# mcahny/vps

Measured on NVIDIA H100. Metric: FuseTrack frame pairs/s on synthetic 1024x2048 pairs, higher is better.
Workload: dtype f32 (wgmma: 3 split-f16 products per MAC, fp32 accumulate promoted to RN register sums)

## Files before the change

### vps_b200/csrc/conv_tc32.cu

```cuda
#include "conv_tc_common.cuh"

namespace {

constexpr int T32_CONV_WARPS = 3;
constexpr int T32_KC = 32;
constexpr int T32_MAX_N = 128;
constexpr int T32_WIDE_MAX_N = 64;
constexpr int t32_threads(int nwg) { return 128 * (nwg + 1); }
constexpr int T32_STAGE_SLOTS = 2;
constexpr int T32_PLANES = 2;

__device__ unsigned int g_tc32_overflow = 0;

struct Tc32Extra {
  int rows;
  int plane_bytes;
  int stage_bytes;
  int b_plane_bytes;
  int dcn;
  int dcn_split_n;
};

struct Dcn32Params {
  const float* x;
// ... 11 lines not shown
              "setmaxnreg counts are multiples of 8 in [24, 256]");

struct Ring32 {
  uint32_t s_base, s_bytes;
  uint32_t a_base, a_bytes;
  uint32_t b_base, b_bytes;
  uint32_t e_base, bias_base;
  uint32_t bar_base;
  __device__ __forceinline__ uint32_t sfull(int s) const { return bar_base + 8u * s; }
  __device__ __forceinline__ uint32_t sempty(int s) const { return bar_base + 8u * (MAX_STAGES + s); }
  __device__ __forceinline__ uint32_t pfull(int s) const { return bar_base + 8u * (2 * MAX_STAGES + s); }
  __device__ __forceinline__ uint32_t pempty(int s) const { return bar_base + 8u * (3 * MAX_STAGES + s); }
  __device__ __forceinline__ uint32_t bfull(int s) const { return bar_base + 8u * (4 * MAX_STAGES + s); }
  __device__ __forceinline__ uint32_t bempty(int s) const { return bar_base + 8u * (5 * MAX_STAGES + s); }
  __device__ __forceinline__ uint32_t unit_ctr() const { return bar_base + 8u * (6 * MAX_STAGES); }
  __device__ __forceinline__ uint32_t rfull(int wg) const { return bar_base + 8u * (6 * MAX_STAGES + 1 + wg); }
};
constexpr int T32_NBAR = 6 * MAX_STAGES;
constexpr int T32_BAR_BYTES = 8 * (T32_NBAR + 2 + 4);
constexpr int t32_box_c(int n) { return n >= 32 ? 32 : 16; }
constexpr int T32_EPI_MAX_N = 64;
constexpr int t32_epi_bytes(int nwg, int bn) { return 64 * nwg * bn * 4 + nwg * bn * 4; }

__device__ __forceinline__ void producer32(const ConvTcParams& p, const Tc32Extra& e, const Ring32& rg, const CUtensorMap* tmA,
                                           const CUtensorMap* tmB) {
  const int ntaps = p.kh * p.kw, kw = p.kw;
  const bool halo = p.halo != 0;
  const uint32_t a_box_bytes = (uint32_t)p.a_box_bytes, b_bytes = (uint32_t)T32_PLANES * (uint32_t)e.b_plane_bytes;
  const int bn = p.block_n;
  int ss = 0, bs = 0;
  uint32_t sphase = 0, bphase = 0;
  for (int tile = blockIdx.x; tile < p.total_tiles; tile += gridDim.x) {
    const TileCoord t = tile_coord(p, tile);
    const int x_base = t.tx * p.tw * p.sw - p.pw_[t.prob];
    const int y_base = t.ty * p.th * p.sh - p.ph_[t.prob];
    const int n0 = t.n_idx * bn;
    for (int cc = 0; cc < p.cin_chunks; ++cc) {
      int r = 0, s = 0;
      for (int tap = 0; tap < ntaps; ++tap) {
        if (!e.dcn && (!halo || tap == 0)) {
          mbar_wait(rg.sempty(ss), sphase ^ 1);
          if (elect_one()) {
            mbar_expect_tx(rg.sfull(ss), a_box_bytes);
            tma_load_4d(rg.s_base + ss * rg.s_bytes, tmA, rg.sfull(ss), cc * T32_KC, halo ? x_base : x_base + s,
                        halo ? y_base : y_base + r, t.img);
          }
          if (++ss == T32_STAGE_SLOTS) { ss = 0; sphase ^= 1; }
        }
        mbar_wait(rg.bempty(bs), bphase ^ 1);
        if (elect_one()) {
          mbar_expect_tx(rg.bfull(bs), b_bytes);
          tma_load_5d(rg.b_base + bs * rg.b_bytes, tmB, rg.bfull(bs), cc * T32_KC, n0, tap, t.prob, 0);
        }
        if (++bs == p.b_stages) { bs = 0; bphase ^= 1; }
        if (++s == kw) { s = 0; ++r; }
      }
    }
  }
}

__device__ __forceinline__ void converter32(const ConvTcParams& p, const Tc32Extra& e, const Ring32& rg, int ctid, int nthreads) {
  const int ntaps = p.kh * p.kw;
  const int items_per_tile = p.cin_chunks * (p.halo ? 1 : ntaps);
  const int tasks = e.rows * 4;
  int ss = 0, as = 0;
  uint32_t sphase = 0, aphase = 0;
  bool over = false;
  for (int tile = blockIdx.x; tile < p.total_tiles; tile += gridDim.x) {
    for (int it = 0; it < items_per_tile; ++it) {
      mbar_wait(rg.sfull(ss), sphase);
      mbar_wait(rg.pempty(as), aphase ^ 1);
      const uint32_t src = rg.s_base + ss * rg.s_bytes;
      const uint32_t dst = rg.a_base + as * rg.a_bytes;
      for (int task = ctid; task < tasks; task += nthreads) {
        const int r = task >> 2, j = task & 3;
        const uint32_t row_s = src + (uint32_t)r * 128u;
        const uint32_t sw = (uint32_t)(r & 7);
        float v[8];
        asm volatile("ld.shared.v4.f32 {%0, %1, %2, %3}, [%4];" : "=f"(v[0]), "=f"(v[1]), "=f"(v[2]), "=f"(v[3])
                     : "r"(row_s + (((uint32_t)(2 * j) ^ sw) << 4)));
        asm volatile("ld.shared.v4.f32 {%0, %1, %2, %3}, [%4];" : "=f"(v[4]), "=f"(v[5]), "=f"(v[6]), "=f"(v[7])
                     : "r"(row_s + (((uint32_t)(2 * j + 1) ^ sw) << 4)));
        uint32_t hp[4], lp[4];
#pragma unroll
        for (int q = 0; q < 4; ++q) split_pair_f16(v[2 * q], v[2 * q + 1], hp[q], lp[q], over);
        const uint32_t off = (uint32_t)r * 64u + ((((uint32_t)j) ^ ((uint32_t)(r >> 1) & 3u)) << 4);
        const uint32_t pm = dst + off, pl = pm + (uint32_t)e.plane_bytes;
        asm volatile("st.shared.v4.b32 [%0], {%1, %2, %3, %4};" ::"r"(pm), "r"(hp[0]), "r"(hp[1]), "r"(hp[2]), "r"(hp[3]) : "memory");
        asm volatile("st.shared.v4.b32 [%0], {%1, %2, %3, %4};" ::"r"(pl), "r"(lp[0]), "r"(lp[1]), "r"(lp[2]), "r"(lp[3]) : "memory");
      }
      mbar_arrive(rg.sempty(ss));
      asm volatile("fence.proxy.async.shared::cta;" ::: "memory");
      mbar_arrive(rg.pfull(as));
      if (++ss == T32_STAGE_SLOTS) { ss = 0; sphase ^= 1; }
      if (++as == p.a_stages) { as = 0; aphase ^= 1; }
    }
  }
  if (over) atomicAdd(&g_tc32_overflow, 1u);
}


__device__ __forceinline__ void dcn_gather32(const ConvTcParams& p, const Tc32Extra& e, const Dcn32Params& d, const Ring32& rg,
                                             uint32_t setup_base, uint32_t ctr_addr, int gtid) {
  constexpr int NT = 32 * DCN32_GATHER_WARPS;
  const int lane = gtid & 31;
  const int j = lane & 3;
  const int rlog = e.rows == 128 ? 7 : 6, ulog = rlog - 3;
  const int steps_per_tile = p.cin_chunks * 9;
  const uint32_t units_per_tile = (uint32_t)steps_per_tile << ulog;
  const uint32_t a_stages = (uint32_t)p.a_stages;
  uint32_t step_base = 0;
  for (int tile = blockIdx.x; tile < p.total_tiles; tile += gridDim.x) {
    const TileCoord t = tile_coord(p, tile);
    if (gtid == 0) asm volatile("st.volatile.shared.u32 [%0], %1;" ::"r"(ctr_addr), "r"(0u) : "memory");
    for (int item = gtid; item < 9 << rlog; item += NT) {
      const int k = item >> rlog, r = item & ((1 << rlog) - 1);
      const int ty_in = r / p.tw, tx_in = r - ty_in * p.tw;
      dcn_setup_entry(d, setup_base + (uint32_t)item * 32u, t.img, t.ty * p.th + ty_in, t.tx * p.tw + tx_in, k);
// ... 85 lines not shown
  for (int h = 0; h < 2; ++h) {
    const int q = 16 * w + (lane >> 2) + 8 * h;
#pragma unroll
    for (int j = 0; j < N / 8; ++j) {
      const int c = 8 * j + 2 * (lane & 3);
      const uint32_t a = epi_box_addr<N>(box, q, c);
      float b0, b1, r0 = 0.f, r1 = 0.f;
      asm volatile("ld.shared.v2.f32 {%0, %1}, [%2];" : "=f"(b0), "=f"(b1) : "r"(bias_s + 4u * c));
      if (p.res) asm volatile("ld.shared.v2.f32 {%0, %1}, [%2];" : "=f"(r0), "=f"(r1) : "r"(a));
      const float2 v = epi_math(p, d[4 * j + 2 * h], d[4 * j + 2 * h + 1], b0, b1, r0, r1);
      asm volatile("st.shared.v2.f32 [%0], {%1, %2};" ::"r"(a), "f"(v.x), "f"(v.y) : "memory");
    }
  }
  asm volatile("fence.proxy.async.shared::cta;" ::: "memory");
  asm volatile("bar.sync %0, 128;" ::"r"(1 + wg) : "memory");
  const EpiBox eb = epi_box(p, tile, wg);
  if (i == 0 && eb.live) {
#pragma unroll
    for (int b = 0; b < N / BC; ++b) tma_store_4d(tmY, box + (uint32_t)b * (64u * BC * 4u), eb.n0 + b * BC, eb.x0, eb.y0, eb.img);
    asm volatile("cp.async.bulk.commit_group;" ::: "memory");
  }
}

template <int N, bool TMA_EPI>
__device__ __forceinline__ void consumer32(const ConvTcParams& p, const Tc32Extra& e, const Ring32& rg, int wg, int row0,
                                           uint32_t b_off, int c_off, const CUtensorMap* tmY, const CUtensorMap* tmR) {
  constexpr int BC = t32_box_c(N);
  const bool leader = (threadIdx.x & 127) == 0;
  constexpr bool epi_tma = TMA_EPI;
  const uint32_t box = rg.e_base + (uint32_t)wg * (64u * N * 4u), bias_s = rg.bias_base + (uint32_t)wg * (N * 4u);
  const uint32_t rbar = rg.rfull(wg);
  uint32_t rphase = 0;
  const bool halo = p.halo != 0;
  const int ntaps = p.kh * p.kw, kw = p.kw, last_cc = p.cin_chunks - 1;
  const uint32_t a_pitch = halo ? (uint32_t)p.halo_w * 64u : 512u;
  const uint64_t a_hi = desc_hi(64u, a_pitch), b_hi = desc_hi(64u, 512u);
  const uint32_t a_wg = halo ? (uint32_t)(row0 >> 3) * a_pitch : (uint32_t)row0 * 64u;
  const uint32_t plane = (uint32_t)e.plane_bytes, b_plane = (uint32_t)e.b_plane_bytes;
  float acc[N / 2], sum[N / 2];
  int as = 0, bs = 0;
  uint32_t aphase = 0, bphase = 0;
  for (int tile = blockIdx.x; tile < p.total_tiles; tile += gridDim.x) {
    float bias_v = 0.f;
    if (epi_tma) {
      const int c = tile_coord(p, tile).n_idx * N + (threadIdx.x & 127);
      if (p.bias && (threadIdx.x & 127) < N && c < p.cout) bias_v = __ldg(p.bias + c);
    }
#pragma unroll
    for (int i = 0; i < N / 2; ++i) sum[i] = 0.f;
    for (int cc = 0; cc <= last_cc; ++cc) {
      const bool two = cc != last_cc || p.nk_last > 1;
      uint32_t a_item = 0;
      int r = 0, s = 0;
      for (int tap = 0; tap < ntaps; ++tap) {
        if (!halo || tap == 0) {
          mbar_wait(rg.pfull(as), aphase);
          a_item = rg.a_base + as * rg.a_bytes + a_wg;
        }
        mbar_wait(rg.bfull(bs), bphase);
        const uint32_t a_addr = halo ? a_item + (uint32_t)r * a_pitch + (uint32_t)s * 64u : a_item;
        const uint32_t b_addr = rg.b_base + bs * rg.b_bytes + b_off;
        const uint64_t A = desc_at(a_hi, a_addr), A2 = desc_at(a_hi, a_addr + plane);
        const uint64_t B = desc_at(b_hi, b_addr), B2 = desc_at(b_hi, b_addr + b_plane);
        wg::fence();
        wg::Mma<N, true>::run(acc, A2, B, 0u);
        if (two) wg::Mma<N, true>::run(acc, A2 + 2, B + 2, 1u);
        wg::Mma<N, true>::run(acc, A, B2, 1u);
        if (two) wg::Mma<N, true>::run(acc, A + 2, B2 + 2, 1u);
        wg::commit();
        wg::wait<0>();
        wg::fence_regs(acc);
#pragma unroll
        for (int i = 0; i < N / 2; ++i) acc[i] *= T32_LO_INV;
        wg::fence();
        wg::Mma<N, true>::run(acc, A, B, 1u);
        if (two) wg::Mma<N, true>::run(acc, A + 2, B + 2, 1u);
        wg::commit();
        wg::wait<0>();
        wg::fence_regs(acc);
#pragma unroll
        for (int i = 0; i < N / 2; ++i) sum[i] += acc[i];
        const bool item_done = !halo || tap == ntaps - 1;
        if (leader) {
          mbar_arrive(rg.bempty(bs));
          if (item_done) mbar_arrive(rg.pempty(as));
          if (epi_tma && p.res && cc == 0 && tap == 0) {
            asm volatile("cp.async.bulk.wait_group.read 0;" ::: "memory");
            const EpiBox eb = epi_box(p, tile, wg);
            if (eb.live) {
              mbar_expect_tx(rbar, 64u * N * 4u);
#pragma unroll
              for (int b = 0; b < N / BC; ++b)
                tma_load_4d(box + (uint32_t)b * (64u * BC * 4u), tmR, rbar, eb.n0 + b * BC, eb.x0, eb.y0, eb.img);
            } else {
              mbar_arrive(rbar);
            }
          }
        }
        if (item_done && ++as == p.a_stages) { as = 0; aphase ^= 1; }
        if (++bs == p.b_stages) { bs = 0; bphase ^= 1; }
        if (++s == kw) { s = 0; ++r; }
      }
    }
    if (epi_tma) {
      epi_tma32<N>(p, tmY, sum, box, bias_s, bias_v, rbar, rphase, wg, tile);
      if (p.res) rphase ^= 1u;
    } else {
      epi_frag<N, 4>(p, sum, tile, row0, c_off);
    }
  }
  if (epi_tma && leader) asm volatile("cp.async.bulk.wait_group 0;" ::: "memory");
}

template <int NWG, bool TMA_EPI>
__device__ __forceinline__ void consumer32_n(const ConvTcParams& p, const Tc32Extra& e, const Ring32& rg, int wg,
                                             const CUtensorMap* tmY, const CUtensorMap* tmR) {
  switch (p.block_n) {
    case 16: consumer32<16, TMA_EPI>(p, e, rg, wg, 64 * wg, 0u, 0, tmY, tmR); break;
    case 32: consumer32<32, TMA_EPI>(p, e, rg, wg, 64 * wg, 0u, 0, tmY, tmR); break;
    case 64: consumer32<64, TMA_EPI>(p, e, rg, wg, 64 * wg, 0u, 0, tmY, tmR); break;
    default:
      if constexpr (NWG == 2 && !TMA_EPI) consumer32<T32_MAX_N, false>(p, e, rg, wg, 64 * wg, 0u, 0, tmY, tmR);
      else __trap();
      break;
  }
}

__device__ __forceinline__ void init_bars32(const Ring32& rg, uint32_t pfull_count, uint32_t sempty_count, uint32_t consumers) {
  for (int i = threadIdx.x & 31; i < T32_NBAR; i += 32) {
    const int kind = i / MAX_STAGES;
    const uint32_t count = kind == 1 ? sempty_count : (kind == 2 ? pfull_count : ((kind == 3 || kind == 5) ? consumers : 1u));
    mbar_init(rg.bar_base + 8u * i, count);
  }
  if ((threadIdx.x & 31) < 4) mbar_init(rg.rfull(threadIdx.x & 31), 1u);
  asm volatile("fence.mbarrier_init.release.cluster;" ::: "memory");
}

template <int NWG, bool TMA_EPI>
__global__ void __launch_bounds__(t32_threads(NWG), 1)
conv_igemm_tc32_kernel(const __grid_constant__ CUtensorMap tmA, const __grid_constant__ CUtensorMap tmB,
                       const __grid_constant__ CUtensorMap tmY, const __grid_constant__ CUtensorMap tmR, const ConvTcParams p,
                       const Tc32Extra e) {
  extern __shared__ __align__(1024) uint8_t smem_raw[];
  const uint32_t smem_base = (smem_u32(smem_raw) + 1023u) & ~1023u;
  Ring32 rg;
  rg.s_base = smem_base; rg.s_bytes = (uint32_t)e.stage_bytes;
  rg.a_base = rg.s_base + T32_STAGE_SLOTS * rg.s_bytes; rg.a_bytes = (uint32_t)T32_PLANES * (uint32_t)e.plane_bytes;
  rg.b_base = rg.a_base + (uint32_t)p.a_stages * rg.a_bytes; rg.b_bytes = (uint32_t)T32_PLANES * (uint32_t)e.b_plane_bytes;
  rg.e_base = rg.b_base + (uint32_t)p.b_stages * rg.b_bytes;
  rg.bias_base = rg.e_base + (TMA_EPI ? 64u * NWG * (uint32_t)p.block_n * 4u : 0u);
  rg.bar_base = rg.bias_base + (TMA_EPI ? (uint32_t)NWG * (uint32_t)p.block_n * 4u : 0u);
  const int warp = __shfl_sync(0xffffffffu, (int)threadIdx.x >> 5, 0);
  if (warp == 0) init_bars32(rg, 32 * T32_CONV_WARPS, 32 * T32_CONV_WARPS, NWG);
  if (threadIdx.x == 32) {
    asm volatile("prefetch.tensormap [%0];" ::"l"(&tmA) : "memory");
    asm volatile("prefetch.tensormap [%0];" ::"l"(&tmB) : "memory");
    if (TMA_EPI) {
      asm volatile("prefetch.tensormap [%0];" ::"l"(&tmY) : "memory");
      if (p.res) asm volatile("prefetch.tensormap [%0];" ::"l"(&tmR) : "memory");
    }
  }
  __syncthreads();
  asm volatile("griddepcontrol.wait;" ::: "memory");
  asm volatile("griddepcontrol.launch_dependents;" ::: "memory");
  if (warp == 0) producer32(p, e, rg, &tmA, &tmB);
  else if (warp < 4) converter32(p, e, rg, (int)threadIdx.x - 32, 32 * T32_CONV_WARPS);
  else consumer32_n<NWG, TMA_EPI>(p, e, rg, (warp - 4) >> 2, &tmY, &tmR);
}

__global__ void __launch_bounds__(DCN32_THREADS, 1)
dcn_igemm_tc32_kernel(const __grid_constant__ CUtensorMap tmB, const ConvTcParams p, const Tc32Extra e, const Dcn32Params d) {
  extern __shared__ __align__(1024) uint8_t smem_raw[];
  const uint32_t smem_base = (smem_u32(smem_raw) + 1023u) & ~1023u;
  Ring32 rg;
  rg.s_base = smem_base; rg.s_bytes = 0;
  rg.a_base = smem_base; rg.a_bytes = (uint32_t)T32_PLANES * (uint32_t)e.plane_bytes;
  rg.b_base = rg.a_base + (uint32_t)p.a_stages * rg.a_bytes; rg.b_bytes = (uint32_t)T32_PLANES * (uint32_t)e.b_plane_bytes;
  const uint32_t setup_base = rg.b_base + (uint32_t)p.b_stages * rg.b_bytes;
  rg.bar_base = setup_base + dcn32_setup_bytes(e.rows);
  const int warp = __shfl_sync(0xffffffffu, (int)threadIdx.x >> 5, 0);
  if (warp == 0) init_bars32(rg, (uint32_t)e.rows / 8u, 1, 2);
  if (threadIdx.x == 32) asm volatile("prefetch.tensormap [%0];" ::"l"(&tmB) : "memory");
  __syncthreads();
  asm volatile("griddepcontrol.wait;" ::: "memory");
  asm volatile("griddepcontrol.launch_dependents;" ::: "memory");
  if (warp >= 4 && warp < 12) {
    asm volatile("setmaxnreg.inc.sync.aligned.u32 %0;" ::"n"(DCN32_HI_REGS));
    const int wg = (warp - 4) >> 2;
    const int bn = e.dcn_split_n ? p.block_n / 2 : p.block_n;
    const int row0 = e.dcn_split_n ? 0 : 64 * wg, c_off = e.dcn_split_n ? bn * wg : 0;
    const uint32_t b_off = (uint32_t)c_off * 64u;
    switch (bn) {
      case 16: consumer32<16, false>(p, e, rg, wg, row0, b_off, c_off, nullptr, nullptr); break;
      case 32: consumer32<32, false>(p, e, rg, wg, row0, b_off, c_off, nullptr, nullptr); break;
      case 64: consumer32<64, false>(p, e, rg, wg, row0, b_off, c_off, nullptr, nullptr); break;
      default: consumer32<DCN32_MAX_N, false>(p, e, rg, wg, row0, b_off, c_off, nullptr, nullptr); break;
    }
  } else {
    asm volatile("setmaxnreg.dec.sync.aligned.u32 %0;" ::"n"(DCN32_LO_REGS));
    if (warp == 0) producer32(p, e, rg, &tmB, &tmB);
    else dcn_gather32(p, e, d, rg, setup_base, rg.unit_ctr(), warp < 4 ? (int)threadIdx.x - 32 : (int)threadIdx.x - 384 + 96);
  }
}

__global__ void pack_weights_tc32_kernel(const float* __restrict__ src, const float* __restrict__ scale, unsigned short* __restrict__ bm,
                                         unsigned short* __restrict__ bl, int cout, int cin, int kh, int kw, int cout_pad,
                                         int cin_pad, int transposed) {
  const int64_t total = (int64_t)cout_pad * kh * kw * cin_pad;
  bool over = false;
  for (int64_t i = blockIdx.x * (int64_t)blockDim.x + threadIdx.x; i < total; i += (int64_t)gridDim.x * blockDim.x) {
    const float v = packed_weight(src, scale, i, cout, cin, kh, kw, cin_pad, transposed);
    unsigned short h, l;
    split_f16(v, h, l);
    over = over || f16_over(v);
    bm[i] = h;
    bl[i] = l;
  }
  if (over) atomicAdd(&g_tc32_overflow, 1u);
}

inline int64_t plane_elems(int cout, int cin, int kh, int kw) {
  const int64_t cout_pad = (cout + 15) / 16 * 16, cin_pad = (cin + T32_KC - 1) / T32_KC * T32_KC;
  return cout_pad * kh * kw * cin_pad;
}

constexpr int T32_SMEM_BUDGET = 227 * 1024 - 1024 - T32_BAR_BYTES - 64;

struct Tc32Plan {
  int nwg;
  int block_n;
  int halo, tw, th, halo_w, halo_h;
  int rows, stage_bytes, plane_bytes, a_stages, a_side;
  int b_stages;
  int epi_tma;
};

bool tc32_epi_expressible(const vps_conv_args* a, int nprob) {
  if (nprob != 1 || a->oy_mul != 1 || a->ox_mul != 1 || a->y.dtype != VPS_F32) return false;
  const int64_t px = (int64_t)a->oy_off * a->y.w + a->ox_off;
  if ((((uintptr_t)a->y.ptr + px * a->y.cs * 4) & 15) || a->y.cs % 4) return false;
  if (a->res.ptr && (a->res.dtype != VPS_F32 || (((uintptr_t)a->res.ptr + px * a->res.cs * 4) & 15) || a->res.cs % 4))
    return false;
  return true;
}

Tc32Plan tc32_tile(const vps_conv_args* a, int nwg) {
  Tc32Plan g = {};
  g.nwg = nwg;
  const int px = 64 * nwg;
  g.halo = a->sh == 1 && a->sw == 1 && a->kh * a->kw > 1 && a->kh <= 8 && a->kw <= 8;
  g.tw = g.halo ? 8 : patch_tw(a->oh, a->ow, px, a->sh, a->sw);
  g.th = px / g.tw;
  g.halo_w = g.tw + a->kw - 1;
  g.halo_h = g.th + a->kh - 1;
  g.rows = g.halo ? g.halo_h * g.halo_w : px;
  g.stage_bytes = (g.rows * 128 + 1023) / 1024 * 1024;
  g.plane_bytes = (g.rows * 64 + 1023) / 1024 * 1024;
  g.a_stages = g.halo ? 2 : 3;
  g.a_side = T32_STAGE_SLOTS * g.stage_bytes + g.a_stages * T32_PLANES * g.plane_bytes;
  return g;
}

int tc32_plan(const vps_conv_args* a, int nprob, Tc32Plan& out) {
  VPS_CHECK_ARG(nprob >= 1 && nprob <= MAX_PROB, "conv2d_tc32: nprob %d", nprob);
  VPS_CHECK_ARG(a->sh >= 1 && a->sh <= 2 && a->sw >= 1 && a->sw <= 2, "conv2d_tc32: stride must be 1 or 2");
  VPS_CHECK_ARG(a->kh >= 1 && a->kw >= 1 && a->cin >= 1 && a->cout >= 1 && a->oh >= 0 && a->ow >= 0 && a->x.n >= 0,
                "conv2d_tc32: bad geometry (k %dx%d, cin %d, cout %d, out %dx%d)", a->kh, a->kw, a->cin, a->cout, a->oh, a->ow);
  const int sms = vps::num_sms();
  if (sms <= 0) { vps::set_error("no device"); return VPS_E_NODEV; }
  const int cout_pad = (a->cout + 15) / 16 * 16;
  const int steps = (a->cin + T32_KC - 1) / T32_KC * a->kh * a->kw;
  double best = -1.0;
  for (int nwg = 2; nwg <= 4; nwg += 2) {
    Tc32Plan g = tc32_tile(a, nwg);
    const int64_t m_tiles = (int64_t)a->x.n * vps::cdiv(a->oh, g.th) * vps::cdiv(a->ow, g.tw) * nprob;
    const double conv = 2.0 * (g.halo ? (double)g.rows / (a->kh * a->kw) : (double)g.rows);
    for (int bn = 16; bn <= (nwg == 2 ? T32_MAX_N : T32_WIDE_MAX_N) && bn <= cout_pad; bn *= 2) {
      if (cout_pad % bn) continue;
      if (g.a_side + 2 * bn * 64 * T32_PLANES > T32_SMEM_BUDGET) continue;
      const int64_t tiles = m_tiles * (cout_pad / bn);
      const double waves = (double)((tiles + sms - 1) / sms);
      const double step = fmax(fmax(300.0, 1.5 * nwg * bn), fmax((double)(bn * 64 * T32_PLANES) / 56.0, conv));
      const double t = waves * ((double)steps * step + 40.0 * bn + 1500.0);
      if (best < 0 || t < best * 0.999) {
        best = t;
        out = g;
        out.block_n = bn;
      }
    }
  }
  if (best < 0) {
    vps::set_error("conv2d_tc32: ring does not fit (k %dx%d)", a->kh, a->kw);
    return VPS_E_ARG;
  }
  const int eb = t32_epi_bytes(out.nwg, out.block_n), b2 = 2 * T32_PLANES * out.block_n * 64;
  out.epi_tma = 0;
  if (!out.halo && out.block_n <= T32_EPI_MAX_N && tc32_epi_expressible(a, nprob)) {
    if (out.a_side + b2 + eb > T32_SMEM_BUDGET && out.a_stages == 3 &&
        out.a_side - T32_PLANES * out.plane_bytes + b2 + eb <= T32_SMEM_BUDGET) {
      out.a_stages = 2;
      out.a_side -= T32_PLANES * out.plane_bytes;
    }
    out.epi_tma = out.a_side + b2 + eb <= T32_SMEM_BUDGET;
  }
  const int bst = (T32_SMEM_BUDGET - out.a_side - (out.epi_tma ? eb : 0)) / (T32_PLANES * out.block_n * 64);
  out.b_stages = bst > MAX_STAGES ? MAX_STAGES : bst;
  return VPS_OK;
}

struct Dcn32Plan {
  int rows;
  int split_n;
  int bn;
  int block_n;
  int n_tiles;
  int tw, th;
  int a_stages, b_stages, smem;
};
constexpr int DCN32_SMEM_MAX = 132 * 1024;
constexpr double DCN32_UNIT_CLK = 220.0, DCN32_STEP_CLK = 300.0;
// ... 76 lines not shown
  const vps_conv_args* a = &args[0];
  VPS_CHECK_ARG(a->x.dtype == VPS_F32, "conv2d_tc32: x must be fp32");
  VPS_CHECK_ARG(a->x.cs % 4 == 0 && ((uintptr_t)a->x.ptr & 15) == 0, "conv2d_tc32: x not 16B aligned (cs=%d)", a->x.cs);
  VPS_CHECK_ARG(a->cin == a->x.c, "conv2d_tc32: cin %d != x.c %d", a->cin, a->x.c);
  VPS_CHECK_ARG(((uintptr_t)a->w & 127) == 0, "conv2d_tc32: weights not aligned");
  for (int i = 0; i < nprob; ++i) {
    VPS_CHECK_ARG(args[i].w == a->w && args[i].x.ptr == a->x.ptr && args[i].y.ptr == a->y.ptr && args[i].kh == a->kh &&
                      args[i].kw == a->kw && args[i].oh == a->oh && args[i].ow == a->ow && args[i].cout == a->cout &&
                      args[i].bias == a->bias && args[i].act == a->act && args[i].oy_mul == a->oy_mul && args[i].ox_mul == a->ox_mul,
                  "conv2d_tc32_multi: problems must share geometry and the packed weight buffer");
  }
  auto encode = vps::tensor_map_encoder();
  if (!encode) return VPS_E_CUDA;
  Tc32Plan g;
  int st = tc32_plan(a, nprob, g);
  if (st != VPS_OK) return st;
  VPS_CHECK_ARG(g.b_stages >= 2, "conv2d_tc32: ring does not fit (%d x %d px halo, bn %d)", g.halo_h, g.halo_w, g.block_n);
  ConvTcParams p = {};
  Tc32Extra e = {};
  p.bk = T32_KC;
  const int cin_pad = (a->cin + T32_KC - 1) / T32_KC * T32_KC;
  const int cout_pad = (a->cout + 15) / 16 * 16;
  p.n_img = a->x.n; p.oh = a->oh; p.ow = a->ow;
  const bool halo = g.halo != 0;
  p.halo = g.halo;
  p.tw = g.tw; p.th = g.th;
  p.halo_w = g.halo_w;
  const int halo_h = g.halo_h;
  e.rows = g.rows;
  p.a_box_bytes = e.rows * 128;
  e.stage_bytes = g.stage_bytes;
  e.plane_bytes = g.plane_bytes;
  p.a_stage_bytes = T32_PLANES * e.plane_bytes;
  p.tiles_x = vps::cdiv(a->ow, p.tw); p.tiles_y = vps::cdiv(a->oh, p.th);
  p.kh = a->kh; p.kw = a->kw; p.sh = a->sh; p.sw = a->sw;
  p.cin_chunks = cin_pad / T32_KC;
  const int rem = a->cin - (p.cin_chunks - 1) * T32_KC;
  p.nk_last = (rem + 15) / 16;
  const int ntaps = a->kh * a->kw;
  p.a_stages = g.a_stages;
  const int block_n = g.block_n;
  p.block_n = block_n; p.n_tiles_n = cout_pad / block_n;
  e.b_plane_bytes = block_n * 64;
  p.b_stages = g.b_stages;
  p.nprob = nprob;
  p.tiles_per_prob = p.n_img * p.tiles_y * p.tiles_x * p.n_tiles_n;
  p.total_tiles = p.tiles_per_prob * nprob;
  st = set_problems(p, args, nprob, "conv2d_tc32");
  if (st != VPS_OK) return st;
  if (p.total_tiles == 0) return VPS_OK;

  CUtensorMap tmA, tmB;
  if (!vps::encode_nhwc(&tmA, a->x, CU_TENSOR_MAP_DATA_TYPE_FLOAT32, T32_KC, halo ? p.halo_w : p.tw * a->sw,
                        halo ? halo_h : p.th * a->sh, a->sw, a->sh, CU_TENSOR_MAP_SWIZZLE_128B, CU_TENSOR_MAP_L2_PROMOTION_L2_128B,
                        "conv2d_tc32: encode A"))
    return VPS_E_CUDA;
  const int64_t n_plane = (int64_t)cout_pad * ntaps * cin_pad;
  {
    cuuint64_t dims[5] = {(cuuint64_t)cin_pad, (cuuint64_t)cout_pad, (cuuint64_t)ntaps, (cuuint64_t)nprob, T32_PLANES};
    cuuint64_t strides[4] = {(cuuint64_t)ntaps * cin_pad * 2, (cuuint64_t)cin_pad * 2, (cuuint64_t)n_plane * 2,
                             (cuuint64_t)n_plane * nprob * 2};
    cuuint32_t box[5] = {(cuuint32_t)T32_KC, (cuuint32_t)block_n, 1, 1, T32_PLANES};
    cuuint32_t estr[5] = {1, 1, 1, 1, 1};
    CUresult r = encode(&tmB, CU_TENSOR_MAP_DATA_TYPE_UINT16, 5, (void*)a->w, dims, strides, box, estr, CU_TENSOR_MAP_INTERLEAVE_NONE,
                        CU_TENSOR_MAP_SWIZZLE_64B, CU_TENSOR_MAP_L2_PROMOTION_L2_256B, CU_TENSOR_MAP_FLOAT_OOB_FILL_NONE);
    if (r != CUDA_SUCCESS) { vps::set_error("conv2d_tc32: encode B failed (%d)", (int)r); return VPS_E_CUDA; }
  }
  CUtensorMap tmY = {}, tmR = {};
  if (g.epi_tma) {
    const int bc = t32_box_c(block_n), box_w = p.tw < 64 ? p.tw : 64;
    const int64_t px = (int64_t)a->oy_off * a->y.w + a->ox_off;
    for (int m = 0; m < (a->res.ptr ? 2 : 1); ++m) {
      const vps_tensor& t = m ? a->res : a->y;
      vps_tensor v = t;
      v.ptr = (float*)t.ptr + px * t.cs; v.n = a->x.n; v.h = a->oh; v.w = a->ow; v.c = a->cout;
      if (!vps::encode_nhwc(m ? &tmR : &tmY, v, CU_TENSOR_MAP_DATA_TYPE_FLOAT32, bc, box_w, 64 / box_w, 1, 1,
                            bc == 32 ? CU_TENSOR_MAP_SWIZZLE_128B : CU_TENSOR_MAP_SWIZZLE_64B, CU_TENSOR_MAP_L2_PROMOTION_L2_128B,
                            m ? "conv2d_tc32: encode residual" : "conv2d_tc32: encode output", &t))
        return VPS_E_CUDA;
    }
  }
  const int smem = g.a_side + p.b_stages * T32_PLANES * e.b_plane_bytes + (g.epi_tma ? t32_epi_bytes(g.nwg, block_n) : 0) + 1024 +
                   T32_BAR_BYTES;
#define VPS_TC32_LAUNCH(NWG, EPI)                                                                                              \
  launch_persistent<conv_igemm_tc32_kernel<NWG, EPI>>(p.total_tiles, t32_threads(NWG), smem, stream, "conv2d_tc32", tmA, tmB, tmY, \
                                                      tmR, p, e)
  if (g.nwg == 4) return g.epi_tma ? VPS_TC32_LAUNCH(4, true) : VPS_TC32_LAUNCH(4, false);
  return g.epi_tma ? VPS_TC32_LAUNCH(2, true) : VPS_TC32_LAUNCH(2, false);
#undef VPS_TC32_LAUNCH
}

extern "C" int vps_conv2d_tc32(const vps_conv_args* a, void* stream) { return vps_conv2d_tc32_multi(a, 1, stream); }

extern "C" int vps_conv2d_tc32_plan(const vps_conv_args* a, int nprob, int* plan) {
  Tc32Plan g;
  const int st = tc32_plan(a, nprob, g);
  if (st != VPS_OK) return st;
  plan[0] = g.nwg; plan[1] = g.block_n; plan[2] = g.tw; plan[3] = g.th; plan[4] = g.halo; plan[5] = g.epi_tma;
  return VPS_OK;
}


extern "C" int vps_deform_conv_tc32(const vps_tensor* x, const vps_tensor* offset, const void* w, int cout, const vps_tensor* y,
                                    void* stream) {
  VPS_CHECK_ARG(x->dtype == VPS_F32 && offset->dtype == VPS_F32 && offset->c >= 18, "deform_conv_tc32: dtypes");
  VPS_CHECK_ARG(x->c % T32_KC == 0 && x->cs % 8 == 0 && ((uintptr_t)x->ptr & 31) == 0,
                "deform_conv_tc32: x must have cin %% 32 == 0 and 32-byte aligned pixel rows (256-bit sampling loads)");
  VPS_CHECK_ARG(offset->n == x->n && offset->h == x->h && offset->w == x->w && y->n == x->n && y->h == x->h && y->w == x->w &&
                    y->c == cout, "deform_conv_tc32: shapes");
  VPS_CHECK_ARG((int64_t)x->n * x->h * x->w * x->cs < (1ll << 31), "deform_conv_tc32: tensor too large for 32-bit offsets");
  VPS_CHECK_ARG(((uintptr_t)w & 127) == 0, "deform_conv_tc32: weights not aligned");
  auto encode = vps::tensor_map_encoder();
  if (!encode) return VPS_E_CUDA;
  VPS_CHECK_ARG(y->dtype == VPS_F32, "deform_conv_tc32: y must be fp32");
  Dcn32Plan g;
  const int st = dcn32_plan(x->n, x->h, x->w, x->c, cout, g);
  if (st != VPS_OK) return st;
  const int cout_pad = (cout + 15) / 16 * 16;
  ConvTcParams p = {};
  Tc32Extra e = {};
  p.bk = T32_KC; p.nprob = 1;
// ... 49 lines not shown
```

### vps_b200/ops.py

```python
import ctypes as C
import os

import torch

from . import _lib
from ._lib import (ACT_LRELU, ACT_NONE, ACT_RELU, ACT_SIGMOID, VPS_BF16, VPS_F32, VpsConvArgs, VpsError,
                   VpsTensor, check, lib)

_DT = {torch.float32: VPS_F32, torch.bfloat16: VPS_BF16}

PROFILE = None
_NOTE = {"flops": 0, "tag": ""}
SCOPE = [""]
_real_lib = lib


class _ProfLib(object):
    def __getattr__(self, name):
        f = getattr(_real_lib(), name)
        if PROFILE is None or not name.startswith("vps_") or name in ("vps_last_error", "vps_launch_count", "vps_packed_tc_bytes"):
            return f

        def w(*a):
            s, e = torch.cuda.Event(enable_timing=True), torch.cuda.Event(enable_timing=True)
# ... 200 lines not shown
    f32 = x.dtype == torch.float32
    for i in range(n):
        a = _conv_args(x, pws[i], y, 1, 0, act, slope, None, False, out_scale, oh, ow, omaps[i], pads[i])
        a.cin_gran = gran
        a.w = shared32.data_ptr() if f32 else pws[i].tc(gran).data_ptr()
        arr[i] = a
    if PROFILE is not None:
        _NOTE["flops"] = 2 * x.shape[0] * arr[0].oh * arr[0].ow * pws[0].cout * pws[0].cin * arr[0].kh * arr[0].kw * n
        _NOTE["tag"] = "%dx%d x%d phases %d->%d @%dx%d" % (arr[0].kh, arr[0].kw, n, pws[0].cin, pws[0].cout, arr[0].oh, arr[0].ow)
    if f32:
        check(lib().vps_conv2d_tc32_multi(arr, n, stream()), "conv2d_tc32_multi")
    else:
        check(lib().vps_conv2d_tc_multi(arr, n, stream()), "conv2d_tc_multi")
    return y


def conv2d_tc32_plan(x, pws, stride=1, pad=0, oh=None, ow=None, pads=None, y=None, res=None, omaps=None):
    pws = pws if isinstance(pws, (list, tuple)) else [pws]
    n = len(pws)
    arr = (VpsConvArgs * n)()
    for i in range(n):
        arr[i] = _conv_args(x, pws[i], x if y is None else y, stride, pad, ACT_NONE, 0.1, res, False, 1.0, oh, ow,
                            omaps[i] if omaps is not None else (1, 0, 1, 0), pads[i] if pads is not None else None)
    plan = (C.c_int * 6)()
    check(_real_lib().vps_conv2d_tc32_plan(arr, n, plan), "conv2d_tc32_plan")
    return dict(nwg=plan[0], block_n=plan[1], tw=plan[2], th=plan[3], halo=plan[4], epilogue="tma" if plan[5] else "frag")


def correlation(f1, f2, out, pad, max_disp, stride1, stride2, act=ACT_NONE, slope=0.1, impl=None):
    fn = {None: "vps_correlation", "tc": "vps_correlation_tc", "simt": "vps_correlation_simt", "tc32": "vps_correlation_tc32"}[impl]
    if PROFILE is not None:
        d = 2 * (max_disp // stride2) + 1
        _NOTE["flops"] = 2 * f1.shape[0] * f1.shape[1] * f1.shape[2] * f1.shape[3] * d * d
        _NOTE["tag"] = "corr d%d s%d C%d @%dx%d" % (max_disp, stride2, f1.shape[3], f1.shape[1], f1.shape[2])
    if impl is None and F32_TC[0] and f1.dtype == torch.float32 and f2.dtype == torch.float32 and out.dtype == torch.float32:
        c = f1.shape[3]
        if (c % 64 == 0 and c <= 256 and stride1 == 1 and pad == max_disp and (max_disp, stride2) == (20, 2)
                and vt(f1).cs % 4 == 0 and vt(f2).cs % 4 == 0 and f1.data_ptr() % 16 == 0 and f2.data_ptr() % 16 == 0):
            fn = "vps_correlation_tc32"
    if fn == "vps_correlation_tc32":
        ws = torch.empty(int(lib().vps_correlation_tc32_ws_bytes(C.byref(vt(f1)))), dtype=torch.uint8, device=f1.device)
        off = (-ws.data_ptr()) % 256
        check(lib().vps_correlation_tc32(C.byref(vt(f1)), C.byref(vt(f2)), C.byref(vt(out)), pad, max_disp, stride1, stride2,
                                         act, C.c_float(slope), C.c_void_p(ws.data_ptr() + off), stream()), "correlation_tc32")
        return out
    check(getattr(lib(), fn)(C.byref(vt(f1)), C.byref(vt(f2)), C.byref(vt(out)), pad, max_disp, stride1,
                                stride2, act, C.c_float(slope), stream()), "correlation")
    return out

# ... 266 lines not shown
```

Measured before the change: 16.62.

## Add phase-decomposed halo tiling for stride-2 convolutions in tc32 conv

Result: faster. 17.11, median of 6 (+3.0%).

```diff
diff --git a/vps_b200/csrc/conv_tc32.cu b/vps_b200/csrc/conv_tc32.cu
--- a/vps_b200/csrc/conv_tc32.cu
+++ b/vps_b200/csrc/conv_tc32.cu
@@ -57,10 +57,37 @@
 constexpr int T32_EPI_MAX_N = 64;
 constexpr int t32_epi_bytes(int nwg, int bn) { return 64 * nwg * bn * 4 + nwg * bn * 4; }
 
+constexpr int T32_FLAT = 0, T32_HALO = 1, T32_PHASE = 2;
+
+struct KStep {
+  int cc, ph, r, s, tap;
+  bool first, last;
+};
+template <bool PH>
+__device__ __forceinline__ int kstep_cols(const ConvTcParams& p, int ph) { return PH ? (p.kw - (ph & 1) + 1) >> 1 : p.kw; }
+template <bool PH>
+__device__ __forceinline__ int kstep_rows(const ConvTcParams& p, int ph) { return PH ? (p.kh - (ph >> 1) + 1) >> 1 : p.kh; }
+template <bool PH>
+__device__ __forceinline__ KStep kstep(const ConvTcParams& p, int cc, int ph, int t, int nt, int r, int s) {
+  KStep k;
+  k.cc = cc; k.ph = ph; k.r = r; k.s = s;
+  k.tap = PH ? (2 * r + (ph >> 1)) * p.kw + 2 * s + (ph & 1) : t;
+  k.first = p.halo == T32_FLAT || t == 0;
+  k.last = p.halo == T32_FLAT || t == nt - 1;
+  return k;
+}
+#define T32_FOR_EACH_KSTEP(PH, p, k)                                                                                      \
+  for (int cc_ = 0; cc_ < (p).cin_chunks; ++cc_)                                                                        \
+    for (int ph_ = 0; ph_ < ((PH) ? 4 : 1); ++ph_)                                                                      \
+      for (int ns_ = kstep_cols<PH>(p, ph_), nt_ = kstep_rows<PH>(p, ph_) * ns_, t_ = 0, r_ = 0, s_ = 0; t_ < nt_;     \
+           ++t_, (++s_ == ns_ ? (s_ = 0, ++r_) : 0))                                                                   \
+        for (bool once_ = true; once_; once_ = false)                                                                 \
+          for (const KStep k = kstep<PH>(p, cc_, ph_, t_, nt_, r_, s_); once_; once_ = false)
+
+template <bool PH>
 __device__ __forceinline__ void producer32(const ConvTcParams& p, const Tc32Extra& e, const Ring32& rg, const CUtensorMap* tmA,
                                            const CUtensorMap* tmB) {
-  const int ntaps = p.kh * p.kw, kw = p.kw;
-  const bool halo = p.halo != 0;
+  const bool flat = p.halo == T32_FLAT;
   const uint32_t a_box_bytes = (uint32_t)p.a_box_bytes, b_bytes = (uint32_t)T32_PLANES * (uint32_t)e.b_plane_bytes;
   const int bn = p.block_n;
   int ss = 0, bs = 0;
@@ -70,65 +97,61 @@
     const int x_base = t.tx * p.tw * p.sw - p.pw_[t.prob];
     const int y_base = t.ty * p.th * p.sh - p.ph_[t.prob];
     const int n0 = t.n_idx * bn;
-    for (int cc = 0; cc < p.cin_chunks; ++cc) {
-      int r = 0, s = 0;
-      for (int tap = 0; tap < ntaps; ++tap) {
-        if (!e.dcn && (!halo || tap == 0)) {
+    T32_FOR_EACH_KSTEP(PH, p, k) {
+        if (!e.dcn && k.first) {
+          const int ox = flat ? k.s : (k.ph & 1), oy = flat ? k.r : (k.ph >> 1);
           mbar_wait(rg.sempty(ss), sphase ^ 1);
           if (elect_one()) {
             mbar_expect_tx(rg.sfull(ss), a_box_bytes);
-            tma_load_4d(rg.s_base + ss * rg.s_bytes, tmA, rg.sfull(ss), cc * T32_KC, halo ? x_base : x_base + s,
-                        halo ? y_base : y_base + r, t.img);
+            tma_load_4d(rg.s_base + ss * rg.s_bytes, tmA, rg.sfull(ss), k.cc * T32_KC, x_base + ox, y_base + oy, t.img);
           }
           if (++ss == T32_STAGE_SLOTS) { ss = 0; sphase ^= 1; }
         }
         mbar_wait(rg.bempty(bs), bphase ^ 1);
         if (elect_one()) {
           mbar_expect_tx(rg.bfull(bs), b_bytes);
-          tma_load_5d(rg.b_base + bs * rg.b_bytes, tmB, rg.bfull(bs), cc * T32_KC, n0, tap, t.prob, 0);
+          tma_load_5d(rg.b_base + bs * rg.b_bytes, tmB, rg.bfull(bs), k.cc * T32_KC, n0, k.tap, t.prob, 0);
         }
         if (++bs == p.b_stages) { bs = 0; bphase ^= 1; }
-        if (++s == kw) { s = 0; ++r; }
-      }
-    }
-  }
-}
-
+    }
+  }
+}
+
+template <bool PH>
 __device__ __forceinline__ void converter32(const ConvTcParams& p, const Tc32Extra& e, const Ring32& rg, int ctid, int nthreads) {
-  const int ntaps = p.kh * p.kw;
-  const int items_per_tile = p.cin_chunks * (p.halo ? 1 : ntaps);
   const int tasks = e.rows * 4;
   int ss = 0, as = 0;
   uint32_t sphase = 0, aphase = 0;
   bool over = false;
   for (int tile = blockIdx.x; tile < p.total_tiles; tile += gridDim.x) {
-    for (int it = 0; it < items_per_tile; ++it) {
-      mbar_wait(rg.sfull(ss), sphase);
-      mbar_wait(rg.pempty(as), aphase ^ 1);
-      const uint32_t src = rg.s_base + ss * rg.s_bytes;
-      const uint32_t dst = rg.a_base + as * rg.a_bytes;
-      for (int task = ctid; task < tasks; task += nthreads) {
-        const int r = task >> 2, j = task & 3;
-        const uint32_t row_s = src + (uint32_t)r * 128u;
-        const uint32_t sw = (uint32_t)(r & 7);
-        float v[8];
-        asm volatile("ld.shared.v4.f32 {%0, %1, %2, %3}, [%4];" : "=f"(v[0]), "=f"(v[1]), "=f"(v[2]), "=f"(v[3])
-                     : "r"(row_s + (((uint32_t)(2 * j) ^ sw) << 4)));
-        asm volatile("ld.shared.v4.f32 {%0, %1, %2, %3}, [%4];" : "=f"(v[4]), "=f"(v[5]), "=f"(v[6]), "=f"(v[7])
-                     : "r"(row_s + (((uint32_t)(2 * j + 1) ^ sw) << 4)));
-        uint32_t hp[4], lp[4];
-#pragma unroll
-        for (int q = 0; q < 4; ++q) split_pair_f16(v[2 * q], v[2 * q + 1], hp[q], lp[q], over);
-        const uint32_t off = (uint32_t)r * 64u + ((((uint32_t)j) ^ ((uint32_t)(r >> 1) & 3u)) << 4);
-        const uint32_t pm = dst + off, pl = pm + (uint32_t)e.plane_bytes;
-        asm volatile("st.shared.v4.b32 [%0], {%1, %2, %3, %4};" ::"r"(pm), "r"(hp[0]), "r"(hp[1]), "r"(hp[2]), "r"(hp[3]) : "memory");
-        asm volatile("st.shared.v4.b32 [%0], {%1, %2, %3, %4};" ::"r"(pl), "r"(lp[0]), "r"(lp[1]), "r"(lp[2]), "r"(lp[3]) : "memory");
-      }
-      mbar_arrive(rg.sempty(ss));
-      asm volatile("fence.proxy.async.shared::cta;" ::: "memory");
-      mbar_arrive(rg.pfull(as));
-      if (++ss == T32_STAGE_SLOTS) { ss = 0; sphase ^= 1; }
-      if (++as == p.a_stages) { as = 0; aphase ^= 1; }
+    T32_FOR_EACH_KSTEP(PH, p, k) {
+        if (!k.first) continue;
+        mbar_wait(rg.sfull(ss), sphase);
+        mbar_wait(rg.pempty(as), aphase ^ 1);
+        const uint32_t src = rg.s_base + ss * rg.s_bytes;
+        const uint32_t dst = rg.a_base + as * rg.a_bytes;
+        for (int task = ctid; task < tasks; task += nthreads) {
+          const int r = task >> 2, j = task & 3;
+          const uint32_t row_s = src + (uint32_t)r * 128u;
+          const uint32_t sw = (uint32_t)(r & 7);
+          float v[8];
+          asm volatile("ld.shared.v4.f32 {%0, %1, %2, %3}, [%4];" : "=f"(v[0]), "=f"(v[1]), "=f"(v[2]), "=f"(v[3])
+                       : "r"(row_s + (((uint32_t)(2 * j) ^ sw) << 4)));
+          asm volatile("ld.shared.v4.f32 {%0, %1, %2, %3}, [%4];" : "=f"(v[4]), "=f"(v[5]), "=f"(v[6]), "=f"(v[7])
+                       : "r"(row_s + (((uint32_t)(2 * j + 1) ^ sw) << 4)));
+          uint32_t hp[4], lp[4];
+#pragma unroll
+          for (int q = 0; q < 4; ++q) split_pair_f16(v[2 * q], v[2 * q + 1], hp[q], lp[q], over);
+          const uint32_t off = (uint32_t)r * 64u + ((((uint32_t)j) ^ ((uint32_t)(r >> 1) & 3u)) << 4);
+          const uint32_t pm = dst + off, pl = pm + (uint32_t)e.plane_bytes;
+          asm volatile("st.shared.v4.b32 [%0], {%1, %2, %3, %4};" ::"r"(pm), "r"(hp[0]), "r"(hp[1]), "r"(hp[2]), "r"(hp[3]) : "memory");
+          asm volatile("st.shared.v4.b32 [%0], {%1, %2, %3, %4};" ::"r"(pl), "r"(lp[0]), "r"(lp[1]), "r"(lp[2]), "r"(lp[3]) : "memory");
+        }
+        mbar_arrive(rg.sempty(ss));
+        asm volatile("fence.proxy.async.shared::cta;" ::: "memory");
+        mbar_arrive(rg.pfull(as));
+        if (++ss == T32_STAGE_SLOTS) { ss = 0; sphase ^= 1; }
+        if (++as == p.a_stages) { as = 0; aphase ^= 1; }
     }
   }
   if (over) atomicAdd(&g_tc32_overflow, 1u);
@@ -260,7 +283,7 @@
   }
 }
 
-template <int N, bool TMA_EPI>
+template <int N, bool TMA_EPI, bool PH>
 __device__ __forceinline__ void consumer32(const ConvTcParams& p, const Tc32Extra& e, const Ring32& rg, int wg, int row0,
                                            uint32_t b_off, int c_off, const CUtensorMap* tmY, const CUtensorMap* tmR) {
   constexpr int BC = t32_box_c(N);
@@ -269,8 +292,7 @@
   const uint32_t box = rg.e_base + (uint32_t)wg * (64u * N * 4u), bias_s = rg.bias_base + (uint32_t)wg * (N * 4u);
   const uint32_t rbar = rg.rfull(wg);
   uint32_t rphase = 0;
-  const bool halo = p.halo != 0;
-  const int ntaps = p.kh * p.kw, kw = p.kw, last_cc = p.cin_chunks - 1;
+  const bool halo = p.halo != T32_FLAT;
   const uint32_t a_pitch = halo ? (uint32_t)p.halo_w * 64u : 512u;
   const uint64_t a_hi = desc_hi(64u, a_pitch), b_hi = desc_hi(64u, 512u);
   const uint32_t a_wg = halo ? (uint32_t)(row0 >> 3) * a_pitch : (uint32_t)row0 * 64u;
@@ -286,17 +308,15 @@
     }
 #pragma unroll
     for (int i = 0; i < N / 2; ++i) sum[i] = 0.f;
-    for (int cc = 0; cc <= last_cc; ++cc) {
-      const bool two = cc != last_cc || p.nk_last > 1;
-      uint32_t a_item = 0;
-      int r = 0, s = 0;
-      for (int tap = 0; tap < ntaps; ++tap) {
-        if (!halo || tap == 0) {
+    uint32_t a_item = 0;
+    T32_FOR_EACH_KSTEP(PH, p, k) {
+        const bool two = k.cc + 1 < p.cin_chunks || p.nk_last > 1;
+        if (k.first) {
           mbar_wait(rg.pfull(as), aphase);
           a_item = rg.a_base + as * rg.a_bytes + a_wg;
         }
         mbar_wait(rg.bfull(bs), bphase);
-        const uint32_t a_addr = halo ? a_item + (uint32_t)r * a_pitch + (uint32_t)s * 64u : a_item;
+        const uint32_t a_addr = halo ? a_item + (uint32_t)k.r * a_pitch + (uint32_t)k.s * 64u : a_item;
         const uint32_t b_addr = rg.b_base + bs * rg.b_bytes + b_off;
         const uint64_t A = desc_at(a_hi, a_addr), A2 = desc_at(a_hi, a_addr + plane);
         const uint64_t B = desc_at(b_hi, b_addr), B2 = desc_at(b_hi, b_addr + b_plane);
@@ -318,11 +338,11 @@
         wg::fence_regs(acc);
 #pragma unroll
         for (int i = 0; i < N / 2; ++i) sum[i] += acc[i];
-        const bool item_done = !halo || tap == ntaps - 1;
+        const bool item_done = k.last;
         if (leader) {
           mbar_arrive(rg.bempty(bs));
           if (item_done) mbar_arrive(rg.pempty(as));
-          if (epi_tma && p.res && cc == 0 && tap == 0) {
+          if (epi_tma && p.res && k.cc == 0 && k.tap == 0) {
             asm volatile("cp.async.bulk.wait_group.read 0;" ::: "memory");
             const EpiBox eb = epi_box(p, tile, wg);
             if (eb.live) {
@@ -337,8 +357,6 @@
         }
         if (item_done && ++as == p.a_stages) { as = 0; aphase ^= 1; }
         if (++bs == p.b_stages) { bs = 0; bphase ^= 1; }
-        if (++s == kw) { s = 0; ++r; }
-      }
     }
     if (epi_tma) {
       epi_tma32<N>(p, tmY, sum, box, bias_s, bias_v, rbar, rphase, wg, tile);
@@ -350,15 +368,15 @@
   if (epi_tma && leader) asm volatile("cp.async.bulk.wait_group 0;" ::: "memory");
 }
 
-template <int NWG, bool TMA_EPI>
+template <int NWG, bool TMA_EPI, bool PH>
 __device__ __forceinline__ void consumer32_n(const ConvTcParams& p, const Tc32Extra& e, const Ring32& rg, int wg,
                                              const CUtensorMap* tmY, const CUtensorMap* tmR) {
   switch (p.block_n) {
-    case 16: consumer32<16, TMA_EPI>(p, e, rg, wg, 64 * wg, 0u, 0, tmY, tmR); break;
-    case 32: consumer32<32, TMA_EPI>(p, e, rg, wg, 64 * wg, 0u, 0, tmY, tmR); break;
-    case 64: consumer32<64, TMA_EPI>(p, e, rg, wg, 64 * wg, 0u, 0, tmY, tmR); break;
+    case 16: consumer32<16, TMA_EPI, PH>(p, e, rg, wg, 64 * wg, 0u, 0, tmY, tmR); break;
+    case 32: consumer32<32, TMA_EPI, PH>(p, e, rg, wg, 64 * wg, 0u, 0, tmY, tmR); break;
+    case 64: consumer32<64, TMA_EPI, PH>(p, e, rg, wg, 64 * wg, 0u, 0, tmY, tmR); break;
     default:
-      if constexpr (NWG == 2 && !TMA_EPI) consumer32<T32_MAX_N, false>(p, e, rg, wg, 64 * wg, 0u, 0, tmY, tmR);
+      if constexpr (NWG == 2 && !TMA_EPI) consumer32<T32_MAX_N, false, PH>(p, e, rg, wg, 64 * wg, 0u, 0, tmY, tmR);
       else __trap();
       break;
   }
@@ -374,7 +392,7 @@
   asm volatile("fence.mbarrier_init.release.cluster;" ::: "memory");
 }
 
-template <int NWG, bool TMA_EPI>
+template <int NWG, bool TMA_EPI, bool PH>
 __global__ void __launch_bounds__(t32_threads(NWG), 1)
 conv_igemm_tc32_kernel(const __grid_constant__ CUtensorMap tmA, const __grid_constant__ CUtensorMap tmB,
                        const __grid_constant__ CUtensorMap tmY, const __grid_constant__ CUtensorMap tmR, const ConvTcParams p,
@@ -401,9 +419,9 @@
   __syncthreads();
   asm volatile("griddepcontrol.wait;" ::: "memory");
   asm volatile("griddepcontrol.launch_dependents;" ::: "memory");
-  if (warp == 0) producer32(p, e, rg, &tmA, &tmB);
-  else if (warp < 4) converter32(p, e, rg, (int)threadIdx.x - 32, 32 * T32_CONV_WARPS);
-  else consumer32_n<NWG, TMA_EPI>(p, e, rg, (warp - 4) >> 2, &tmY, &tmR);
+  if (warp == 0) producer32<PH>(p, e, rg, &tmA, &tmB);
+  else if (warp < 4) converter32<PH>(p, e, rg, (int)threadIdx.x - 32, 32 * T32_CONV_WARPS);
+  else consumer32_n<NWG, TMA_EPI, PH>(p, e, rg, (warp - 4) >> 2, &tmY, &tmR);
 }
 
 __global__ void __launch_bounds__(DCN32_THREADS, 1)
@@ -429,14 +447,14 @@
     const int row0 = e.dcn_split_n ? 0 : 64 * wg, c_off = e.dcn_split_n ? bn * wg : 0;
     const uint32_t b_off = (uint32_t)c_off * 64u;
     switch (bn) {
-      case 16: consumer32<16, false>(p, e, rg, wg, row0, b_off, c_off, nullptr, nullptr); break;
-      case 32: consumer32<32, false>(p, e, rg, wg, row0, b_off, c_off, nullptr, nullptr); break;
-      case 64: consumer32<64, false>(p, e, rg, wg, row0, b_off, c_off, nullptr, nullptr); break;
-      default: consumer32<DCN32_MAX_N, false>(p, e, rg, wg, row0, b_off, c_off, nullptr, nullptr); break;
+      case 16: consumer32<16, false, false>(p, e, rg, wg, row0, b_off, c_off, nullptr, nullptr); break;
+      case 32: consumer32<32, false, false>(p, e, rg, wg, row0, b_off, c_off, nullptr, nullptr); break;
+      case 64: consumer32<64, false, false>(p, e, rg, wg, row0, b_off, c_off, nullptr, nullptr); break;
+      default: consumer32<DCN32_MAX_N, false, false>(p, e, rg, wg, row0, b_off, c_off, nullptr, nullptr); break;
     }
   } else {
     asm volatile("setmaxnreg.dec.sync.aligned.u32 %0;" ::"n"(DCN32_LO_REGS));
-    if (warp == 0) producer32(p, e, rg, &tmB, &tmB);
+    if (warp == 0) producer32<false>(p, e, rg, &tmB, &tmB);
     else dcn_gather32(p, e, d, rg, setup_base, rg.unit_ctr(), warp < 4 ? (int)threadIdx.x - 32 : (int)threadIdx.x - 384 + 96);
   }
 }
@@ -467,7 +485,8 @@
 struct Tc32Plan {
   int nwg;
   int block_n;
-  int halo, tw, th, halo_w, halo_h;
+  int halo;
+  int tw, th, halo_w, halo_h;
   int rows, stage_bytes, plane_bytes, a_stages, a_side;
   int b_stages;
   int epi_tma;
@@ -482,19 +501,21 @@
   return true;
 }
 
-Tc32Plan tc32_tile(const vps_conv_args* a, int nwg) {
+Tc32Plan tc32_tile(const vps_conv_args* a, int nwg, int kind) {
   Tc32Plan g = {};
   g.nwg = nwg;
   const int px = 64 * nwg;
-  g.halo = a->sh == 1 && a->sw == 1 && a->kh * a->kw > 1 && a->kh <= 8 && a->kw <= 8;
-  g.tw = g.halo ? 8 : patch_tw(a->oh, a->ow, px, a->sh, a->sw);
+  g.halo = kind;
+  const bool halo = kind != T32_FLAT;
+  const int kh = kind == T32_PHASE ? (a->kh + 1) / 2 : a->kh, kw = kind == T32_PHASE ? (a->kw + 1) / 2 : a->kw;
+  g.tw = halo ? 8 : patch_tw(a->oh, a->ow, px, a->sh, a->sw);
   g.th = px / g.tw;
-  g.halo_w = g.tw + a->kw - 1;
-  g.halo_h = g.th + a->kh - 1;
-  g.rows = g.halo ? g.halo_h * g.halo_w : px;
+  g.halo_w = g.tw + kw - 1;
+  g.halo_h = g.th + kh - 1;
+  g.rows = halo ? g.halo_h * g.halo_w : px;
   g.stage_bytes = (g.rows * 128 + 1023) / 1024 * 1024;
   g.plane_bytes = (g.rows * 64 + 1023) / 1024 * 1024;
-  g.a_stages = g.halo ? 2 : 3;
+  g.a_stages = halo ? 2 : 3;
   g.a_side = T32_STAGE_SLOTS * g.stage_bytes + g.a_stages * T32_PLANES * g.plane_bytes;
   return g;
 }
@@ -507,12 +528,18 @@
   const int sms = vps::num_sms();
   if (sms <= 0) { vps::set_error("no device"); return VPS_E_NODEV; }
   const int cout_pad = (a->cout + 15) / 16 * 16;
-  const int steps = (a->cin + T32_KC - 1) / T32_KC * a->kh * a->kw;
+  const int ntaps = a->kh * a->kw;
+  const int steps = (a->cin + T32_KC - 1) / T32_KC * ntaps;
+  const bool halo = a->sh == 1 && a->sw == 1 && ntaps > 1 && a->kh <= 8 && a->kw <= 8;
+  const bool phase = a->sh == 2 && a->sw == 2 && a->kh >= 2 && a->kw >= 2 && a->kh <= 7 && a->kw <= 7;
+  const int kinds[2] = {halo ? T32_HALO : (phase ? T32_PHASE : T32_FLAT), T32_FLAT};
   double best = -1.0;
+  for (int ki = 0; ki < (phase ? 2 : 1); ++ki)
   for (int nwg = 2; nwg <= 4; nwg += 2) {
-    Tc32Plan g = tc32_tile(a, nwg);
+    Tc32Plan g = tc32_tile(a, nwg, kinds[ki]);
     const int64_t m_tiles = (int64_t)a->x.n * vps::cdiv(a->oh, g.th) * vps::cdiv(a->ow, g.tw) * nprob;
-    const double conv = 2.0 * (g.halo ? (double)g.rows / (a->kh * a->kw) : (double)g.rows);
+    const int items = g.halo == T32_FLAT ? ntaps : (g.halo == T32_HALO ? 1 : 4);
+    const double conv = 2.0 * g.rows * items / ntaps;
     for (int bn = 16; bn <= (nwg == 2 ? T32_MAX_N : T32_WIDE_MAX_N) && bn <= cout_pad; bn *= 2) {
       if (cout_pad % bn) continue;
       if (g.a_side + 2 * bn * 64 * T32_PLANES > T32_SMEM_BUDGET) continue;
@@ -533,7 +560,7 @@
   }
   const int eb = t32_epi_bytes(out.nwg, out.block_n), b2 = 2 * T32_PLANES * out.block_n * 64;
   out.epi_tma = 0;
-  if (!out.halo && out.block_n <= T32_EPI_MAX_N && tc32_epi_expressible(a, nprob)) {
+  if (out.halo != T32_HALO && out.block_n <= T32_EPI_MAX_N && tc32_epi_expressible(a, nprob)) {
     if (out.a_side + b2 + eb > T32_SMEM_BUDGET && out.a_stages == 3 &&
         out.a_side - T32_PLANES * out.plane_bytes + b2 + eb <= T32_SMEM_BUDGET) {
       out.a_stages = 2;
@@ -656,7 +683,7 @@
   const int cin_pad = (a->cin + T32_KC - 1) / T32_KC * T32_KC;
   const int cout_pad = (a->cout + 15) / 16 * 16;
   p.n_img = a->x.n; p.oh = a->oh; p.ow = a->ow;
-  const bool halo = g.halo != 0;
+  const bool halo = g.halo != T32_FLAT;
   p.halo = g.halo;
   p.tw = g.tw; p.th = g.th;
   p.halo_w = g.halo_w;
@@ -685,8 +712,8 @@
   if (p.total_tiles == 0) return VPS_OK;
 
   CUtensorMap tmA, tmB;
-  if (!vps::encode_nhwc(&tmA, a->x, CU_TENSOR_MAP_DATA_TYPE_FLOAT32, T32_KC, halo ? p.halo_w : p.tw * a->sw,
-                        halo ? halo_h : p.th * a->sh, a->sw, a->sh, CU_TENSOR_MAP_SWIZZLE_128B, CU_TENSOR_MAP_L2_PROMOTION_L2_128B,
+  if (!vps::encode_nhwc(&tmA, a->x, CU_TENSOR_MAP_DATA_TYPE_FLOAT32, T32_KC, (halo ? p.halo_w : p.tw) * a->sw,
+                        (halo ? halo_h : p.th) * a->sh, a->sw, a->sh, CU_TENSOR_MAP_SWIZZLE_128B, CU_TENSOR_MAP_L2_PROMOTION_L2_128B,
                         "conv2d_tc32: encode A"))
     return VPS_E_CUDA;
   const int64_t n_plane = (int64_t)cout_pad * ntaps * cin_pad;
@@ -716,11 +743,15 @@
   }
   const int smem = g.a_side + p.b_stages * T32_PLANES * e.b_plane_bytes + (g.epi_tma ? t32_epi_bytes(g.nwg, block_n) : 0) + 1024 +
                    T32_BAR_BYTES;
-#define VPS_TC32_LAUNCH(NWG, EPI)                                                                                              \
-  launch_persistent<conv_igemm_tc32_kernel<NWG, EPI>>(p.total_tiles, t32_threads(NWG), smem, stream, "conv2d_tc32", tmA, tmB, tmY, \
+#define VPS_TC32_LAUNCH(NWG, EPI, PH)                                                                                          \
+  launch_persistent<conv_igemm_tc32_kernel<NWG, EPI, PH>>(p.total_tiles, t32_threads(NWG), smem, stream, "conv2d_tc32", tmA, tmB, tmY, \
                                                       tmR, p, e)
-  if (g.nwg == 4) return g.epi_tma ? VPS_TC32_LAUNCH(4, true) : VPS_TC32_LAUNCH(4, false);
-  return g.epi_tma ? VPS_TC32_LAUNCH(2, true) : VPS_TC32_LAUNCH(2, false);
+  if (g.halo == T32_PHASE) {
+    if (g.nwg == 4) return g.epi_tma ? VPS_TC32_LAUNCH(4, true, true) : VPS_TC32_LAUNCH(4, false, true);
+    return g.epi_tma ? VPS_TC32_LAUNCH(2, true, true) : VPS_TC32_LAUNCH(2, false, true);
+  }
+  if (g.nwg == 4) return g.epi_tma ? VPS_TC32_LAUNCH(4, true, false) : VPS_TC32_LAUNCH(4, false, false);
+  return g.epi_tma ? VPS_TC32_LAUNCH(2, true, false) : VPS_TC32_LAUNCH(2, false, false);
 #undef VPS_TC32_LAUNCH
 }
 
@@ -730,7 +761,8 @@
   Tc32Plan g;
   const int st = tc32_plan(a, nprob, g);
   if (st != VPS_OK) return st;
-  plan[0] = g.nwg; plan[1] = g.block_n; plan[2] = g.tw; plan[3] = g.th; plan[4] = g.halo; plan[5] = g.epi_tma;
+  plan[0] = g.nwg; plan[1] = g.block_n; plan[2] = g.tw; plan[3] = g.th; plan[4] = g.halo == T32_HALO; plan[5] = g.epi_tma;
+  plan[6] = g.halo;
   return VPS_OK;
 }
 
diff --git a/vps_b200/ops.py b/vps_b200/ops.py
--- a/vps_b200/ops.py
+++ b/vps_b200/ops.py
@@ -246,9 +246,10 @@
     for i in range(n):
         arr[i] = _conv_args(x, pws[i], x if y is None else y, stride, pad, ACT_NONE, 0.1, res, False, 1.0, oh, ow,
                             omaps[i] if omaps is not None else (1, 0, 1, 0), pads[i] if pads is not None else None)
-    plan = (C.c_int * 6)()
+    plan = (C.c_int * 7)()
     check(_real_lib().vps_conv2d_tc32_plan(arr, n, plan), "conv2d_tc32_plan")
-    return dict(nwg=plan[0], block_n=plan[1], tw=plan[2], th=plan[3], halo=plan[4], epilogue="tma" if plan[5] else "frag")
+    return dict(nwg=plan[0], block_n=plan[1], tw=plan[2], th=plan[3], halo=plan[4], epilogue="tma" if plan[5] else "frag",
+                kind=("flat", "halo", "phase")[plan[6]])
 
 
 def correlation(f1, f2, out, pad, max_disp, stride1, stride2, act=ACT_NONE, slope=0.1, impl=None):
```
